# Niccolo-Ajroldi/plainLM

Hardware: AMD Instinct MI355X
Metric: tokens/sec fwd+bwd (160M, seq=1024, bf16) (higher is better)
Workload: dtype bf16

## Files before the change

### plainlm_amd/csrc/gemm_big.hip

```cpp
#include <stdlib.h>

#include <type_traits>
#include <utility>

#include "plm_device.h"

#include <initializer_list>

typedef __attribute__((address_space(3))) void lds_void_t;
typedef const __attribute__((address_space(1))) void gbl_void_t;

__device__ __forceinline__ void big_dma16(const void* gsrc, void* lds_wave_base) {
  __builtin_amdgcn_global_load_lds((gbl_void_t*)gsrc, (lds_void_t*)lds_wave_base, 16, 0, 0);
}
__device__ __forceinline__ int big_swz(int row, int chunk) { return row * 128 + ((chunk ^ ((row >> 1) & 7)) << 4); }

template <int N>
__device__ __forceinline__ void wait_vm() {
#ifdef PLM_DBG_DRAIN
  asm volatile("s_waitcnt vmcnt(0)" ::: "memory");
#else
  asm volatile("s_waitcnt vmcnt(%0)" ::"n"(N) : "memory");
#endif
}
template <int N0, int N1>
__device__ __forceinline__ void wait_vm_sel(int flag) {
#ifdef PLM_DBG_DRAIN
  asm volatile("s_waitcnt vmcnt(0)" ::: "memory");
  return;
#endif
  asm volatile("s_cmp_lg_u32 %0, 0\n\ts_cbranch_scc1 1f\n\ts_waitcnt vmcnt(%1)\n\ts_branch 2f\n1:\n\ts_waitcnt vmcnt(%2)\n2:" ::"s"(flag), "n"(N0), "n"(N1)
               : "memory", "scc");
}
template <int N0, int N1, int N2>
__device__ __forceinline__ void wait_vm_sel3(int flag) {
#ifdef PLM_DBG_DRAIN
  asm volatile("s_waitcnt vmcnt(0)" ::: "memory");
  return;
#endif
  asm volatile("s_cmp_lg_u32 %0, 0\n\ts_cbranch_scc1 1f\n\ts_waitcnt vmcnt(%1)\n\ts_branch 3f\n1:\n\ts_cmp_lg_u32 %0, 1\n\ts_cbranch_scc1 2f\n\ts_waitcnt vmcnt(%2)\n\t"
               "s_branch 3f\n2:\n\ts_waitcnt vmcnt(%3)\n3:" ::"s"(flag), "n"(N0), "n"(N1), "n"(N2)
               : "memory", "scc");
}
__device__ __forceinline__ void phase_barrier() { asm volatile("s_waitcnt lgkmcnt(0)\n\ts_barrier" ::: "memory"); }

#define BIG_GROUP_M 4

static int g_num_cus = 0;
static int g_cu_reserve = 0;

static int persistent_slots() {
  const int n = g_num_cus - g_cu_reserve;
  return n < 8 ? 8 : n;
}

extern "C" int plm_set_cu_reserve(int n) {
  if (n < 0 || n > 128) {
    plm_set_error("plm_set_cu_reserve: n=%d out of range 0..128", n);
    return PLM_E_INVALID;
  }
  g_cu_reserve = n;
  return PLM_OK;
}

static bool ensure_num_cus() {
  if (g_num_cus == 0) {
    int dev = 0;
    hipDeviceProp_t prop;
    if (hipGetDevice(&dev) != hipSuccess || hipGetDeviceProperties(&prop, dev) != hipSuccess) return false;
    g_num_cus = prop.multiProcessorCount > 0 ? prop.multiProcessorCount : 256;
  }
  return true;
}

static double round_efficiency(int64_t tiles, int slots) {
  const int64_t rounds = (tiles + slots - 1) / slots;
  return (double)tiles / (double)(rounds * slots);
}

struct HybridArgs {
  int rfull;
  int nchunks;
  int L;
  float* slabs;
};

struct EpiArgs {
  uint16_t* act;
  int64_t ldact;
  const float* rcos;
  const float* rsin;
  int T, rope_cols;
};

template <class F, int... U>
__device__ __forceinline__ void nt_for_units(F& f, std::integer_sequence<int, U...>) {
  (f(std::integral_constant<int, U>{}), ...);
}
template <int NA, int NBF, int BF0>
struct NtOvlPlan {
  static constexpr int NPASS = (NBF + 1) / 2, NUNIT = NA * NPASS;
  static constexpr int pass_blocks(int u) { const int p0 = (u % NPASS) * 2; return NBF - p0 < 2 ? NBF - p0 : 2; }
  static constexpr int stores(int u) { return 2 * pass_blocks(u); }
  static constexpr int ready(int u) {
    const int mf = u / NPASS, p0 = (u % NPASS) * 2, nb = pass_blocks(u);
    const int h[2] = {(2 * mf) / NA, (2 * mf + 1) / NA};
    const bool b[2] = {p0 < BF0, p0 + nb - 1 >= BF0};
    int r = 0;
    for (int i = 0; i < 2; ++i)
      for (int j = 0; j < 2; ++j)
        if (b[j]) {
          const int ph = h[i] == 0 ? (j == 0 ? 1 : 2) : (j == 1 ? 3 : 4);
          r = ph > r ? ph : r;
        }
    return r;
  }
  static constexpr int slot(int u) {
    bool taken[6] = {false, false, false, false, false, false};
    int slot_u = 5;
    for (int r = 1; r <= 4; ++r)
      for (int v = 0; v < NUNIT; ++v)
        if (ready(v) == r) {
          int sl = 5;
          for (int c = r + 1; c <= 4; ++c)
            if (!taken[c]) {
              sl = c;
              break;
            }
          if (sl < 5) taken[sl] = true;
          if (v == u) slot_u = sl;
        }
    return slot_u;
  }
  static constexpr int stores_in_slot(int sl) {
    int n = 0;
    for (int u = 0; u < NUNIT; ++u)
      if (slot(u) == sl) n += stores(u);
    return n;
  }
  static constexpr int unit_in_slot(int sl) {
    for (int u = 0; u < NUNIT; ++u)
      if (slot(u) == sl) return u;
    return -1;
  }
};
static_assert(NtOvlPlan<2, 3, 2>::slot(0) == 2 && NtOvlPlan<2, 3, 2>::slot(1) == 3 && NtOvlPlan<2, 3, 2>::slot(3) == 4 && NtOvlPlan<2, 3, 2>::slot(2) == 5,
              "256x192: (A0,B0) (A0,B1) (A1,B1) leave in phases 2 3 4, (A1,B0) behind the loop");
static_assert(NtOvlPlan<4, 2, 1>::slot(0) == 3 && NtOvlPlan<4, 2, 1>::slot(1) == 4 && NtOvlPlan<4, 2, 1>::slot(2) == 5 && NtOvlPlan<4, 2, 1>::slot(3) == 5,
              "256x256: the two pieces of A half 0 leave in phases 3 and 4");
static_assert(NtOvlPlan<1, 3, 2>::slot(1) == 4 && NtOvlPlan<1, 3, 2>::slot(0) == 5, "128x192: the B1 pass leaves in phase 4");

template <int BM, int BN, int WM, int WN, bool HYB = false, bool GLU = false, bool GLUB = false, bool ROPE = false>
__global__ __launch_bounds__(512, 2) void gemm_nt_big_kernel(const uint16_t* __restrict__ A, int64_t lda,
                                                             const uint16_t* __restrict__ B, int64_t ldb,
                                                             uint16_t* __restrict__ C, int64_t ldc, int M, int N, int K,
                                                             const float* __restrict__ alpha_dev, int tiles_m, int tiles_n,
                                                             HybridArgs hyb, EpiArgs ea) {
  uint16_t* const act = ea.act;
  const int64_t ldact = ea.ldact;
  static_assert(!(GLU || GLUB) || (BM == 256 && BN == 256 && WN == 4 && !HYB), "GLU epilogues: 256x256 tiles, whole-K items");
  static_assert(!(GLU && GLUB), "one epilogue at a time");
  constexpr int TM = BM / WM, TN = BN / WN;
  static_assert(WM * WN == 8 && (TN == 64 || TN == 96) && (TM == 128 || TM == 64 || TM == 32), "unsupported geometry");
  constexpr int AH = TM / 2;
  constexpr int NA = AH / 16;
  constexpr int BF0 = TN / 32 - 1, NBF = BF0 + 1;
  constexpr int A_ROWS = BM / 2, B0_ROWS = WN * 32 * BF0, B1_ROWS = WN * 32;
  constexpr int A_HT = A_ROWS * 128, B0_HT = B0_ROWS * 128, B1_HT = B1_ROWS * 128;
  constexpr int STAGE = 2 * A_HT + B0_HT + B1_HT;
  constexpr int A_DMA = A_ROWS / 64, B0_DMA = B0_ROWS / 64, B1_DMA = B1_ROWS / 64;
  static_assert(B0_DMA >= B1_DMA && B1_DMA >= 1, "half-tiles are whole DMA rounds of the workgroup");
  constexpr int OFF_A0 = 0, OFF_B0 = A_HT, OFF_B1 = A_HT + B0_HT, OFF_A1 = A_HT + B0_HT + B1_HT;
  constexpr int D_P4 = 2 * A_DMA + B0_DMA + 2 * B1_DMA;
  constexpr int D_P1 = 3 * A_DMA + B0_DMA + B1_DMA;
  constexpr int D_P2 = 3 * A_DMA + B0_DMA + B1_DMA;
  constexpr int NS = NA * 2 * NBF * (GLUB ? 2 : 1) + (GLU ? NA * 2 : 0);
  static_assert(D_P1 + NS < 64, "vmcnt is a 6-bit counter");
#ifndef PLM_NT_OVL
#define PLM_NT_OVL 1
#endif
  constexpr bool OVL = PLM_NT_OVL && !HYB && !GLU && !GLUB && !ROPE;
  using OP = NtOvlPlan<NA, NBF, BF0>;
  constexpr int NPASS = OP::NPASS, NUNIT = OP::NUNIT;
  constexpr int OVS_2 = OVL ? OP::stores_in_slot(2) : 0, OVS_3 = OVL ? OP::stores_in_slot(3) : 0, OVS_4 = OVL ? OP::stores_in_slot(4) : 0;
  static_assert(OVS_2 + OVS_3 + OVS_4 + (OVL ? OP::stores_in_slot(5) : NS) == NS, "every unit has a slot");
  static_assert(D_P4 + NS < 64, "vmcnt is a 6-bit counter");
  __shared__ __attribute__((aligned(1024))) char smem[2 * STAGE + 8 * 4096];

  const int t = threadIdx.x, lane = t & 63;
  const int wave = __builtin_amdgcn_readfirstlane(t >> 6);
  const int wm = wave / WN, wn = wave % WN;
  const bool grp1 = (wave >> 2) != 0;
  if (wave >= 4) __builtin_amdgcn_s_setprio(1);
  const int l15 = lane & 15, q = lane >> 4;
  const int rfull = HYB ? hyb.rfull : tiles_m;
  const int n_full = rfull * tiles_n;
  const int nkt = K / 64;
  const int g_total = HYB ? (tiles_m - rfull) * tiles_n * nkt : 0;
  const int ntiles = n_full + (HYB ? hyb.nchunks : 0);
  char* epi = smem + 2 * STAGE + wave * 4096;

  struct Cur {
    int item, g, gend;
  };
  auto cur_init = [&](Cur& c, int item) {
    c.item = item;
    c.g = c.gend = 0;
    if (HYB && item >= n_full && item < ntiles) {
      c.g = (item - n_full) * hyb.L;
      c.gend = min(g_total, c.g + hyb.L);
    }
  };
  auto take = [&](Cur& c, int& m0, int& n0, int& kbeg, int& kend, int& sidx) {
    if (!HYB || c.item < n_full) {
      const int group_size = BIG_GROUP_M * tiles_n;
      const int group = c.item / group_size;
      const int first_m = group * BIG_GROUP_M;
      const int gm = min(rfull - first_m, BIG_GROUP_M);
      const int in_group = c.item - group * group_size;
      m0 = (first_m + in_group % gm) * BM;
      n0 = (in_group / gm) * BN;
      kbeg = 0;
      kend = K;
      sidx = -1;
      cur_init(c, c.item + gridDim.x);
    } else {
      const int t = c.g / nkt;
      const int k0 = c.g - t * nkt;
      const int k1 = min(nkt, k0 + (c.gend - c.g));
      m0 = (rfull + t / tiles_n) * BM;
      n0 = (t % tiles_n) * BN;
      kbeg = k0 * 64;
      kend = k1 * 64;
      sidx = (c.item - n_full) - (t * nkt) / hyb.L;
      c.g += k1 - k0;
      if (c.g >= c.gend) cur_init(c, c.item + gridDim.x);
    }
  };

  unsigned oa[2][A_DMA], ob[2][B0_DMA];
  const uint16_t* s_ab = A;
  const uint16_t* s_bb = B;
  const uint16_t* s_ak = A;
  const uint16_t* s_bk = B;
  auto set_ptrs = [&](int m0, int n0) {
    s_ab = A + (int64_t)m0 * lda;
    s_bb = B + (int64_t)(GLU ? n0 / 2 : n0) * ldb;
#pragma unroll
    for (int h = 0; h < 2; ++h) {
#pragma unroll
      for (int i = 0; i < A_DMA; ++i) {
        const int r = (i * 8 + wave) * 8 + (lane >> 3);
        const int chunk = (lane & 7) ^ ((r >> 1) & 7);
        const int m = min((r / AH) * TM + h * AH + (r % AH), M - 1 - m0);
        oa[h][i] = (unsigned)(((int64_t)m * lda + chunk * 8) * 2);
      }
#pragma unroll
      for (int i = 0; i < (h ? B1_DMA : B0_DMA); ++i) {
        const int r = (i * 8 + wave) * 8 + (lane >> 3);
        const int chunk = (lane & 7) ^ ((r >> 1) & 7);
        const int rw = h ? 32 : 32 * BF0;
        const int n = GLU ? h * (N / 2) + r : min((r / rw) * TN + h * 32 * BF0 + (r % rw), N - 1 - n0);
        ob[h][i] = (unsigned)(((int64_t)n * ldb + chunk * 8) * 2);
      }
    }
  };
  auto issue_a = [&](int h, char* stage, int k0) {
    char* dst = stage + (h ? OFF_A1 : OFF_A0);
#pragma unroll
    for (int i = 0; i < A_DMA; ++i) {
      (void)k0;
      big_dma16(reinterpret_cast<const char*>(s_ak) + oa[h][i], dst + (i * 8 + wave) * 1024);
    }
  };
  auto issue_b = [&](int h, char* stage, int k0) {
    char* dst = stage + (h ? OFF_B1 : OFF_B0);
#pragma unroll
    for (int i = 0; i < B0_DMA; ++i) {
      if (i >= (h ? B1_DMA : B0_DMA)) continue;
      (void)k0;
      big_dma16(reinterpret_cast<const char*>(s_bk) + ob[h][i], dst + (i * 8 + wave) * 1024);
    }
  };
  auto frag16 = [&](const char* ht, int row, int ks) -> bf16x8_t {
    return *reinterpret_cast<const bf16x8_t*>(ht + big_swz(row, ks * 4 + q));
  };

  const int first = xcd_remap(blockIdx.x, gridDim.x);
  if (first >= ntiles) return;
  Cur sc;
  cur_init(sc, first);
  int s_k = 0, s_kend = 0;
  int s_item = first;
  auto open_piece = [&]() {
    s_item = sc.item;
    if (s_item < ntiles) {
      int m0, n0, sp_;
      take(sc, m0, n0, s_k, s_kend, sp_);
      set_ptrs(m0, n0);
      s_ak = s_ab + s_k;
      s_bk = s_bb + s_k;
    } else {
      s_k -= 64;
      s_ak -= 64;
      s_bk -= 64;
    }
  };
  int s_st = 0;
  auto advance_staged = [&]() {
    s_k += 64;
    s_ak += 64;
    s_bk += 64;
    s_st ^= 1;
    if (s_k >= s_kend) open_piece();
  };
  open_piece();

  float alpha = alpha_dev ? *alpha_dev : 1.f;
  asm volatile("; alpha pinned" : "+v"(alpha));

  {
    issue_a(0, smem, s_k);
    issue_b(0, smem, s_k);
    issue_b(1, smem, s_k);
    issue_a(1, smem, s_k);
    advance_staged();
  }
  {
    issue_a(0, smem + STAGE, s_k);
    issue_b(0, smem + STAGE, s_k);
    issue_b(1, smem + STAGE, s_k);
    wait_vm<D_P4>();
  }
  phase_barrier();

  int st = 0;
  bool credit = false;
  int credit_i = 0;
  Cur cc;
  cur_init(cc, first);
  while (cc.item < ntiles) {
    int m0 = 0, n0 = 0, kbeg = 0, kend = K, split = -1;
    if (HYB) take(cc, m0, n0, kbeg, kend, split);
    const int nk = HYB ? (kend - kbeg) / 64 : nkt;
    f32x4_t acc4[2 * NA][2 * NBF];
#pragma unroll
    for (int i = 0; i < 2 * NA; ++i)
#pragma unroll
      for (int j = 0; j < 2 * NBF; ++j)
#pragma unroll
        for (int r = 0; r < 4; ++r) acc4[i][j][r] = 0.f;

    auto unit_write = [&](auto utag) {
      constexpr int u = decltype(utag)::value, mf = u / NPASS, p0 = (u % NPASS) * 2, nb = OP::pass_blocks(u);
#pragma unroll
      for (int bq = 0; bq < nb; ++bq) {
        const int bh = p0 + bq;
#pragma unroll
        for (int sr = 0; sr < 2; ++sr)
#pragma unroll
          for (int sc = 0; sc < 2; ++sc) {
            bf16x4_t o;
#pragma unroll
            for (int e = 0; e < 4; ++e) o[e] = f2bf(acc4[2 * mf + sr][bh * 2 + sc][e]);
            const int row = sr * 16 + l15, c = bq * 4 + sc * 2 + (q >> 1);
            *reinterpret_cast<bf16x4_t*>(epi + row * 128 + ((c ^ (row & 7)) << 4) + (q & 1) * 8) = o;
          }
      }
    };
    auto unit_store = [&](auto utag, auto interior, int m0, int n0) {
      constexpr int u = decltype(utag)::value, mf = u / NPASS, p0 = (u % NPASS) * 2, nb = OP::pass_blocks(u);
      const int mrow0 = m0 + wm * TM + mf * 32;
      bf16x8_t v[2 * nb];
#pragma unroll
      for (int it = 0; it < 2 * nb; ++it) {
        const int c = it * 64 + lane;
        const int row = nb == 2 ? c >> 3 : c >> 2, ch = nb == 2 ? c & 7 : c & 3;
        v[it] = *reinterpret_cast<const bf16x8_t*>(epi + row * 128 + ((ch ^ (row & 7)) << 4));
      }
#pragma unroll
      for (int it = 0; it < 2 * nb; ++it) {
        const int c = it * 64 + lane;
        const int row = nb == 2 ? c >> 3 : c >> 2, ch = nb == 2 ? c & 7 : c & 3;
        const int gm = mrow0 + row;
        const int gn = n0 + wn * TN + p0 * 32 + ch * 8;
        if (decltype(interior)::value || (gm < M && gn < N)) st_c_bf16x8(C + (int64_t)gm * ldc + gn, v[it]);
      }
    };

    auto ktile = [&](auto lasttag, int m0, int n0) {
      constexpr bool LASTOVL = decltype(lasttag)::value;
      const char* cur = smem + st * STAGE;
      bf16x8_t a6[NA][2], b06[2 * BF0][2], b16[2][2];
      auto end_phase = [&](auto wtag, auto w2tag) {
        constexpr int W = decltype(wtag)::value, W2 = decltype(w2tag)::value;
        if (LASTOVL) wait_vm<W>();
        else if (OVL) wait_vm_sel3<W, W + NS, W + W2>(credit_i);
        else wait_vm_sel<W, W + NS>(credit_i);
        phase_barrier();
      };
      using std::integral_constant;
      auto slot_write = [&](auto sltag) {
        constexpr int u = OP::unit_in_slot(decltype(sltag)::value);
        if constexpr (LASTOVL && u >= 0) unit_write(integral_constant<int, (u >= 0 ? u : 0)>{});
      };
      auto slot_store = [&](auto sltag) {
        constexpr int u = OP::unit_in_slot(decltype(sltag)::value);
        if constexpr (LASTOVL && u >= 0) {
          asm volatile("s_waitcnt lgkmcnt(0)" ::: "memory");
          unit_store(integral_constant<int, (u >= 0 ? u : 0)>{}, std::true_type{}, m0, n0);
        }
      };
      constexpr int S2 = LASTOVL ? OVS_2 : 0, S4 = LASTOVL ? OVS_2 + OVS_3 + OVS_4 : 0;

      issue_a(1, smem + s_st * STAGE, s_k);
      advance_staged();
#pragma unroll
      for (int ks = 0; ks < 2; ++ks) {
#pragma unroll
        for (int j = 0; j < 2 * BF0; ++j) b06[j][ks] = frag16(cur + OFF_B0, wn * BF0 * 32 + j * 16 + l15, ks);
#pragma unroll
        for (int f = 0; f < NA; ++f) a6[f][ks] = frag16(cur + OFF_A0, wm * AH + f * 16 + l15, ks);
      }
      if (grp1) end_phase(integral_constant<int, D_P1>{}, integral_constant<int, NS>{});
#pragma unroll
      for (int ks = 0; ks < 2; ++ks)
#pragma unroll
        for (int f = 0; f < NA; ++f)
#pragma unroll
          for (int j = 0; j < 2 * BF0; ++j) acc4[f][j] = mfma16(b06[j][ks], a6[f][ks], acc4[f][j]);
      if (!grp1) end_phase(integral_constant<int, D_P1>{}, integral_constant<int, NS>{});

      issue_a(0, smem + s_st * STAGE, s_k);
#pragma unroll
      for (int ks = 0; ks < 2; ++ks)
#pragma unroll
        for (int c = 0; c < 2; ++c) b16[c][ks] = frag16(cur + OFF_B1, wn * 32 + c * 16 + l15, ks);
      slot_write(integral_constant<int, 2>{});
      if (grp1) end_phase(integral_constant<int, D_P2>{}, integral_constant<int, NS>{});
#pragma unroll
      for (int ks = 0; ks < 2; ++ks)
#pragma unroll
        for (int f = 0; f < NA; ++f)
#pragma unroll
          for (int c = 0; c < 2; ++c) acc4[f][2 * BF0 + c] = mfma16(b16[c][ks], a6[f][ks], acc4[f][2 * BF0 + c]);
      slot_store(integral_constant<int, 2>{});
      if (!grp1) end_phase(integral_constant<int, D_P2 + S2>{}, integral_constant<int, NS>{});

      issue_b(0, smem + s_st * STAGE, s_k);
#pragma unroll
      for (int ks = 0; ks < 2; ++ks)
#pragma unroll
        for (int f = 0; f < NA; ++f) a6[f][ks] = frag16(cur + OFF_A1, wm * AH + f * 16 + l15, ks);
      slot_write(integral_constant<int, 3>{});
      if (grp1) end_phase(integral_constant<int, D_P4 - B1_DMA + S2>{}, integral_constant<int, NS - OVS_2>{});
#pragma unroll
      for (int ks = 0; ks < 2; ++ks)
#pragma unroll
        for (int f = 0; f < NA; ++f)
#pragma unroll
          for (int c = 0; c < 2; ++c) acc4[NA + f][2 * BF0 + c] = mfma16(b16[c][ks], a6[f][ks], acc4[NA + f][2 * BF0 + c]);
      slot_store(integral_constant<int, 3>{});

      issue_b(1, smem + s_st * STAGE, s_k);
      slot_write(integral_constant<int, 4>{});
#pragma unroll
      for (int ks = 0; ks < 2; ++ks)
#pragma unroll
        for (int f = 0; f < NA; ++f)
#pragma unroll
          for (int j = 0; j < 2 * BF0; ++j) acc4[NA + f][j] = mfma16(b06[j][ks], a6[f][ks], acc4[NA + f][j]);
      slot_store(integral_constant<int, 4>{});
      if (!grp1) end_phase(integral_constant<int, D_P4 + S4>{}, integral_constant<int, NS - OVS_2>{});
      credit = false;
      credit_i = 0;
      st ^= 1;
    };

    bool ovl = false;
    if (OVL) {
      Cur peek = cc;
      int pm0, pn0, pk0, pk1, psp;
      take(peek, pm0, pn0, pk0, pk1, psp);
      ovl = __builtin_amdgcn_readfirstlane(nk >= 2 && alpha_dev == nullptr && pm0 + BM <= M && pn0 + BN <= N);
    }
    {
      const int nloop = ovl ? nk - 1 : nk;
      for (int kt = 0; kt < nloop; ++kt) ktile(std::false_type{}, 0, 0);
    }
    if (OVL && ovl) {
      Cur peek = cc;
      int pm0, pn0, pk0, pk1, psp;
      take(peek, pm0, pn0, pk0, pk1, psp);
      ktile(std::true_type{}, pm0, pn0);
    }

    if (!HYB) take(cc, m0, n0, kbeg, kend, split);
    if (HYB && split >= 0) {
      const int mrem = M - rfull * BM;
      float* slab = hyb.slabs + ((int64_t)split * mrem - (int64_t)rfull * BM) * N;
#pragma unroll
      for (int f = 0; f < 2 * NA; ++f) {
        const int gm = m0 + wm * TM + f * 16 + l15;
        if (gm >= M) continue;
#pragma unroll
        for (int j = 0; j < 2 * NBF; ++j) {
          const int gn = n0 + wn * TN + j * 16 + 4 * q;
          if (gn >= N) continue;
          *reinterpret_cast<f32x4_t*>(slab + (int64_t)gm * N + gn) = acc4[f][j];
        }
      }
      continue;
    }
    if (HYB || alpha_dev != nullptr) {
#pragma unroll
      for (int i = 0; i < 2 * NA; ++i)
#pragma unroll
        for (int j = 0; j < 2 * NBF; ++j) acc4[i][j] *= alpha;
    }
    if constexpr (OVL) {
      auto drain = [&](auto utag) {
        constexpr int u = decltype(utag)::value;
        if (ovl && OP::slot(u) != 5) return;
        unit_write(utag);
        asm volatile("s_waitcnt lgkmcnt(0)" ::: "memory");
        unit_store(utag, std::false_type{}, m0, n0);
        asm volatile("s_waitcnt lgkmcnt(0)" ::: "memory");
      };
      nt_for_units(drain, std::make_integer_sequence<int, NUNIT>{});
      credit = m0 + BM <= M && n0 + BN <= N;
      credit_i = __builtin_amdgcn_readfirstlane(credit ? (ovl ? 2 : 1) : 0);
      continue;
    }
#pragma unroll
    for (int mf = 0; mf < NA; ++mf) {
      const int mrow0 = m0 + wm * TM + mf * 32;
      if (GLUB) {
        const uint16_t* u = act;
#pragma unroll
        for (int sr = 0; sr < 2; ++sr) {
          const int gm_l = min(mrow0 + sr * 16 + l15, M - 1);
          const int fi = 2 * mf + sr;
#pragma unroll
          for (int bq = 0; bq < 2; ++bq)
#pragma unroll
            for (int sc = 0; sc < 2; ++sc) {
              const int gn = n0 + wn * TN + bq * 32 + sc * 16 + 4 * q;
              const bf16x4_t xv = ld_bf16x4(u + (int64_t)gm_l * ldact + gn);
              const bf16x4_t zv = ld_bf16x4(u + (int64_t)gm_l * ldact + N + gn);
              bf16x4_t dxo, dzo;
#pragma unroll
              for (int e = 0; e < 4; ++e) {
                const float gf = bf2f(f2bf(acc4[fi][bq * 2 + sc][e]));
                const float xf = bf2f(xv[e]), zf = bf2f(zv[e]);
                const float sig = plm_sigmoid(xf);
                const bf16_t sv = f2bf(xf * sig);
                const bf16_t ds = f2bf(gf * zf);
                dzo[e] = f2bf(gf * bf2f(sv));
                dxo[e] = f2bf(bf2f(ds) * (sig * (1.f + xf * (1.f - sig))));
              }
              const int c = bq * 4 + sc * 2 + (q >> 1);
              *reinterpret_cast<bf16x4_t*>(epi + l15 * 128 + ((c ^ (l15 & 7)) << 4) + (q & 1) * 8) = dxo;
              *reinterpret_cast<bf16x4_t*>(epi + (16 + l15) * 128 + ((c ^ (l15 & 7)) << 4) + (q & 1) * 8) = dzo;
            }
          asm volatile("s_waitcnt lgkmcnt(0)" ::: "memory");
#pragma unroll
          for (int it = 0; it < 4; ++it) {
            const int c = it * 64 + lane;
            const int row = c >> 3, ch = c & 7;
            const bf16x8_t v = *reinterpret_cast<const bf16x8_t*>(epi + row * 128 + ((ch ^ (row & 7)) << 4));
            const int gm = mrow0 + sr * 16 + (row & 15);
            if (gm < M) st_c2_bf16x8(C + (int64_t)gm * ldc + (row >> 4) * N + n0 + wn * TN + ch * 8, v);
          }
          asm volatile("s_waitcnt lgkmcnt(0)" ::: "memory");
        }
        continue;
      }
#pragma unroll
      for (int p0 = 0; p0 < NBF; p0 += 2) {
        const int nb = NBF - p0 < 2 ? NBF - p0 : 2;
#pragma unroll
        for (int bq = 0; bq < 2; ++bq) {
          if (bq >= nb) continue;
          const int bh = p0 + bq;
#pragma unroll
          for (int sr = 0; sr < 2; ++sr)
#pragma unroll
            for (int sc = 0; sc < 2; ++sc) {
              bf16x4_t o;
#pragma unroll
              for (int e = 0; e < 4; ++e) o[e] = f2bf(acc4[2 * mf + sr][bh * 2 + sc][e]);
              const int row = sr * 16 + l15, c = bq * 4 + sc * 2 + (q >> 1);
              *reinterpret_cast<bf16x4_t*>(epi + row * 128 + ((c ^ (row & 7)) << 4) + (q & 1) * 8) = o;
            }
        }
        asm volatile("s_waitcnt lgkmcnt(0)" ::: "memory");
#pragma unroll
        for (int it = 0; it < 4; ++it) {
          if (it >= 2 * nb) continue;
          const int c = it * 64 + lane;
          const int row = nb == 2 ? c >> 3 : c >> 2, ch = nb == 2 ? c & 7 : c & 3;
          const bf16x8_t v = *reinterpret_cast<const bf16x8_t*>(epi + row * 128 + ((ch ^ (row & 7)) << 4));
          const int gm = mrow0 + row;
          const int gn = GLU ? (ch >> 2) * (N / 2) + n0 / 2 + wn * 32 + (ch & 3) * 8 : n0 + wn * TN + p0 * 32 + ch * 8;
          if (ROPE) {
            if (gm < M && gn < ea.rope_cols) {
              const int tab = (gm % ea.T) * 32 + ((gn & 63) >> 1);
              st_c2_bf16x8(C + (int64_t)gm * ldc + gn, rope8(v, *reinterpret_cast<const f32x4_t*>(ea.rcos + tab),
                                                          *reinterpret_cast<const f32x4_t*>(ea.rsin + tab), 1.f));
              continue;
            }
          }
          if (gm < M && gn < N) st_c_bf16x8(C + (int64_t)gm * ldc + gn, v);
        }
        asm volatile("s_waitcnt lgkmcnt(0)" ::: "memory");
      }
      if (GLU) {
#pragma unroll
        for (int sr = 0; sr < 2; ++sr)
#pragma unroll
          for (int sc = 0; sc < 2; ++sc) {
            const int fi = 2 * mf + sr;
            bf16x4_t o;
#pragma unroll
            for (int e = 0; e < 4; ++e) o[e] = plm_swiglu_bf16(f2bf(acc4[fi][sc][e]), f2bf(acc4[fi][2 + sc][e]));
            const int row = sr * 16 + l15, c = sc * 2 + (q >> 1);
            *reinterpret_cast<bf16x4_t*>(epi + row * 128 + ((c ^ (row & 7)) << 4) + (q & 1) * 8) = o;
          }
        asm volatile("s_waitcnt lgkmcnt(0)" ::: "memory");
#pragma unroll
        for (int it = 0; it < 2; ++it) {
          const int c = it * 64 + lane;
          const int row = c >> 2, ch = c & 3;
          const bf16x8_t v = *reinterpret_cast<const bf16x8_t*>(epi + row * 128 + ((ch ^ (row & 7)) << 4));
          const int gm = mrow0 + row;
          if (gm < M) st_c2_bf16x8(act + (int64_t)gm * ldact + n0 / 2 + wn * 32 + ch * 8, v);
        }
        asm volatile("s_waitcnt lgkmcnt(0)" ::: "memory");
      }
    }
    credit = m0 + BM <= M && n0 + BN <= N;
    credit_i = __builtin_amdgcn_readfirstlane(credit ? 1 : 0);
  }
  wait_vm<0>();
}

#define PLM_TN_GROUP_MAX 48
struct TnGroup {
  const uint16_t* A[PLM_TN_GROUP_MAX];
  const uint16_t* B[PLM_TN_GROUP_MAX];
  int lda[PLM_TN_GROUP_MAX], ldb[PLM_TN_GROUP_MAX];
  int M[PLM_TN_GROUP_MAX], N[PLM_TN_GROUP_MAX], tiles_n[PLM_TN_GROUP_MAX];
  int tile_base[PLM_TN_GROUP_MAX + 1];
  int count;
  int n_full;
  int splits;
  int L;
};
struct TnGroupOut {
  float* C[PLM_TN_GROUP_MAX];
  const float* alpha[PLM_TN_GROUP_MAX];
  int ldc[PLM_TN_GROUP_MAX];
  int accumulate[PLM_TN_GROUP_MAX];
};

__device__ __forceinline__ int tn_rot(int k) { return 2 * (k & 3) + ((k >> 3) & 1); }

template <bool GROUPED = false>
__global__ __launch_bounds__(512, 2) void gemm_tn_big_kernel(const uint16_t* __restrict__ A, int64_t lda,
                                                             const uint16_t* __restrict__ B, int64_t ldb, float* __restrict__ C,
                                                             int64_t ldc, float* __restrict__ slabs, int M, int N, int K, int kchunk,
                                                             int splits, int rfull, int accumulate,
                                                             const float* __restrict__ alpha_dev, int tiles_m, int tiles_n, TnGroup grp,
                                                             TnGroupOut gout) {
  constexpr int BM = 256, BN = 256, WN = 4;
  constexpr int TM = 128, TN = 64, AH = 64, AF = 2, NA = 2 * AF;
  constexpr int HT = 64 * 256;
  constexpr int STAGE = 4 * HT;
  constexpr int OFF_A0 = 0, OFF_B0 = HT, OFF_B1 = 2 * HT, OFF_A1 = 3 * HT;
  constexpr int W_ALL = 10;
  __shared__ __attribute__((aligned(1024))) char smem[2 * STAGE];

  const int t = threadIdx.x, lane = t & 63;
  const int wave = __builtin_amdgcn_readfirstlane(t >> 6);
  const int wm = wave / WN, wn = wave % WN;
  const bool grp1 = (wave >> 2) != 0;
#ifndef PLM_NO_PRIO_HALF_TN
  if (wave >= 4) __builtin_amdgcn_s_setprio(1);
#endif
  const int t16 = lane & 15;
  const int q = lane >> 4;
  const int n_full = rfull * tiles_n;
  const int n_rem = tiles_m * tiles_n - n_full;
  const int nkt = K / 64;
  const int g_ntl = GROUPED ? grp.tile_base[grp.count] : 0, g_nrem = GROUPED ? g_ntl - grp.n_full : 0;
  const int nitems = GROUPED ? grp.n_full + g_nrem * grp.splits : n_full + n_rem * splits;
  int c_prob = 0, c_tile = 0;

  auto coords = [&](int item, int& i0, int& j0, int& kbeg, int& kend, int& split) {
    int tile;
    if (GROUPED) {
      int t, lo, hi2;
      if (item < grp.n_full) {
        split = -1;
        t = item;
        lo = 0;
        hi2 = nkt;
      } else {
        const int j = item - grp.n_full;
        split = j / g_nrem;
        t = grp.n_full + (j - split * g_nrem);
        lo = min(nkt, split * grp.L);
        hi2 = min(nkt, (split + 1) * grp.L);
      }
      kbeg = kend = 0;
      i0 = j0 = 0;
      if (hi2 <= lo) return;
      t = __builtin_amdgcn_readfirstlane(t);
      int pidx = 0;
#pragma unroll
      for (int q = 1; q < PLM_TN_GROUP_MAX; ++q)
        if (q < grp.count && t >= grp.tile_base[q]) pidx = q;
      pidx = __builtin_amdgcn_readfirstlane(pidx);
      const int local = t - grp.tile_base[pidx];
      i0 = (local / grp.tiles_n[pidx]) * BM;
      j0 = (local % grp.tiles_n[pidx]) * BN;
      kbeg = lo * 64;
      kend = hi2 * 64;
      c_prob = pidx;
      c_tile = t;
      return;
    }
    if (item < n_full) {
      split = -1;
      tile = item;
      kbeg = 0;
      kend = K;
    } else {
      const int j = item - n_full;
      split = j / n_rem;
      tile = n_full + (j - split * n_rem);
      kbeg = min(K, split * kchunk);
      kend = min(K, kbeg + kchunk);
    }
    i0 = (tile / tiles_n) * BM;
    j0 = (tile % tiles_n) * BN;
  };

  unsigned pa[2][2], pb[2][2];
  const uint16_t* s_ap = A;
  const uint16_t* s_bp = B;
  int64_t s_lda = lda, s_ldb = ldb;
  auto set_ptrs = [&](int item) {
    int i0, j0, kbeg, kend, split;
    coords(item, i0, j0, kbeg, kend, split);
    const uint16_t* Ap = GROUPED ? grp.A[c_prob] : A;
    const uint16_t* Bp = GROUPED ? grp.B[c_prob] : B;
    const int Mp = GROUPED ? grp.M[c_prob] : M, Np = GROUPED ? grp.N[c_prob] : N;
    if (GROUPED) {
      s_lda = (int64_t)grp.lda[c_prob];
      s_ldb = (int64_t)grp.ldb[c_prob];
    }
    s_ap = Ap;
    s_bp = Bp;
#pragma unroll
    for (int i = 0; i < 2; ++i) {
      const int row = (i * 8 + wave) * 4 + (lane >> 4);
      const int pp = (lane & 15) >> 1, half16 = lane & 1;
      const int cb = (pp - tn_rot(row)) & 7;
      const int c = cb * 16 + half16 * 8;
#pragma unroll
      for (int h = 0; h < 2; ++h) {
        const int ci = i0 + (c / AH) * TM + h * AH + (c % AH);
        const int cj = j0 + (c / 32) * TN + h * 32 + (c % 32);
        pa[h][i] = (unsigned)(((int64_t)row * s_lda + min(ci, Mp - 8)) * 2);
        pb[h][i] = (unsigned)(((int64_t)row * s_ldb + min(cj, Np - 8)) * 2);
      }
    }
  };
  const unsigned smem_u = __builtin_amdgcn_readfirstlane(lds_addr_u32(smem));
  auto issue = [&](const uint16_t* base, const unsigned (&off)[2], int64_t ld, unsigned dst, int k0) {
    const uint16_t* kb = base + (int64_t)k0 * ld;
#pragma unroll
    for (int i = 0; i < 2; ++i) dma16_saddr_u32(kb, off[i], dst + (i * 8 + wave) * 1024);
  };
  auto tr_frag16 = [&](const char* ht, int c0, int ks) -> bf16x8_t {
    const int row = ks * 32 + q * 8 + (t16 >> 2);
    const char* p = ht + row * 256 + (((c0 >> 4) + tn_rot(row)) & 7) * 32 + (t16 & 3) * 8;
    return join_tr(lds_read_tr16(p), lds_read_tr16(p + 4 * 256));
  };

  const int first = xcd_remap(blockIdx.x, gridDim.x);
  if (first >= nitems) return;
  float alpha = alpha_dev ? *alpha_dev : 1.f;
  asm volatile("; alpha pinned" : "+v"(alpha));

  int s_item = first, s_k = 0, s_kend = 0;
  auto open_item = [&]() {
    while (s_item < nitems) {
      int i0, j0, kbeg, kend, split;
      coords(s_item, i0, j0, kbeg, kend, split);
      if (kend > kbeg) {
        s_k = kbeg;
        s_kend = kend;
        set_ptrs(s_item);
        return;
      }
      s_item += gridDim.x;
    }
  };
  int s_st = 0;
  auto advance_staged = [&]() {
    s_k += 64;
    s_st ^= 1;
    if (s_k >= s_kend) {
      s_item += gridDim.x;
      open_item();
    }
  };
  open_item();
  if (s_item < nitems) {
    issue(s_ap, pa[0], s_lda, smem_u + OFF_A0, s_k);
    issue(s_bp, pb[0], s_ldb, smem_u + OFF_B0, s_k);
    issue(s_bp, pb[1], s_ldb, smem_u + OFF_B1, s_k);
    issue(s_ap, pa[1], s_lda, smem_u + OFF_A1, s_k);
    advance_staged();
  }
  if (s_item < nitems) {
    issue(s_ap, pa[0], s_lda, smem_u + STAGE + OFF_A0, s_k);
    issue(s_bp, pb[0], s_ldb, smem_u + STAGE + OFF_B0, s_k);
    issue(s_bp, pb[1], s_ldb, smem_u + STAGE + OFF_B1, s_k);
    wait_vm<W_ALL>();
  } else {
    wait_vm<0>();
// ... 549 lines not shown
```

Before: 1.066 million.

## Defer last epilogue unit store into next tile's first k-iteration

In the overlapped persistent GEMM, the epilogue unit in slot 5 was written to LDS and stored after the k-loop. It is now packed into bf16 registers and carried over to the next tile, where its LDS write and global store are issued during the first k-tile's MFMA phase. The vmcnt wait thresholds for that first k-tile are adjusted to account for the deferred stores. This hides tail epilogue latency behind compute, at the cost of extra live registers and more complex counter bookkeeping.

```diff
diff --git a/plainlm_amd/csrc/gemm_big.hip b/plainlm_amd/csrc/gemm_big.hip
--- a/plainlm_amd/csrc/gemm_big.hip
+++ b/plainlm_amd/csrc/gemm_big.hip
@@ -184,6 +184,13 @@
   constexpr int NPASS = OP::NPASS, NUNIT = OP::NUNIT;
   constexpr int OVS_2 = OVL ? OP::stores_in_slot(2) : 0, OVS_3 = OVL ? OP::stores_in_slot(3) : 0, OVS_4 = OVL ? OP::stores_in_slot(4) : 0;
   static_assert(OVS_2 + OVS_3 + OVS_4 + (OVL ? OP::stores_in_slot(5) : NS) == NS, "every unit has a slot");
+#ifndef PLM_NT_DEFER
+#define PLM_NT_DEFER 1
+#endif
+  constexpr int DU = OVL ? OP::unit_in_slot(5) : -1;
+  constexpr bool DEFER = PLM_NT_DEFER && OVL && DU >= 0 && OP::stores_in_slot(5) == OP::stores(DU < 0 ? 0 : DU);
+  constexpr int DS = DEFER ? OP::stores(DU) : 0;
+  constexpr int DNB = DEFER ? OP::pass_blocks(DU) : 1;
   static_assert(D_P4 + NS < 64, "vmcnt is a 6-bit counter");
   __shared__ __attribute__((aligned(1024))) char smem[2 * STAGE + 8 * 4096];
 
@@ -337,6 +344,8 @@
   int st = 0;
   bool credit = false;
   int credit_i = 0;
+  bf16x4_t dpk[DNB * 4];
+  int dpend = 0, dm0 = 0, dn0 = 0;
   Cur cc;
   cur_init(cc, first);
   while (cc.item < ntiles) {
@@ -351,21 +360,48 @@
 #pragma unroll
         for (int r = 0; r < 4; ++r) acc4[i][j][r] = 0.f;
 
+    auto unit_pack = [&](auto utag, bf16x4_t* o) {
+      constexpr int u = decltype(utag)::value, mf = u / NPASS, p0 = (u % NPASS) * 2, nb = OP::pass_blocks(u);
+#pragma unroll
+      for (int bq = 0; bq < nb; ++bq)
+#pragma unroll
+        for (int sr = 0; sr < 2; ++sr)
+#pragma unroll
+          for (int sc = 0; sc < 2; ++sc)
+#pragma unroll
+            for (int e = 0; e < 4; ++e) o[(bq * 2 + sr) * 2 + sc][e] = f2bf(acc4[2 * mf + sr][(p0 + bq) * 2 + sc][e]);
+    };
+    auto unit_put = [&](auto utag, const bf16x4_t* o) {
+      constexpr int nb = OP::pass_blocks(decltype(utag)::value);
+#pragma unroll
+      for (int bq = 0; bq < nb; ++bq)
+#pragma unroll
+        for (int sr = 0; sr < 2; ++sr)
+#pragma unroll
+          for (int sc = 0; sc < 2; ++sc) {
+            const int row = sr * 16 + l15, c = bq * 4 + sc * 2 + (q >> 1);
+            *reinterpret_cast<bf16x4_t*>(epi + row * 128 + ((c ^ (row & 7)) << 4) + (q & 1) * 8) = o[(bq * 2 + sr) * 2 + sc];
+          }
+    };
     auto unit_write = [&](auto utag) {
       constexpr int u = decltype(utag)::value, mf = u / NPASS, p0 = (u % NPASS) * 2, nb = OP::pass_blocks(u);
-#pragma unroll
-      for (int bq = 0; bq < nb; ++bq) {
-        const int bh = p0 + bq;
-#pragma unroll
-        for (int sr = 0; sr < 2; ++sr)
-#pragma unroll
-          for (int sc = 0; sc < 2; ++sc) {
-            bf16x4_t o;
-#pragma unroll
-            for (int e = 0; e < 4; ++e) o[e] = f2bf(acc4[2 * mf + sr][bh * 2 + sc][e]);
-            const int row = sr * 16 + l15, c = bq * 4 + sc * 2 + (q >> 1);
-            *reinterpret_cast<bf16x4_t*>(epi + row * 128 + ((c ^ (row & 7)) << 4) + (q & 1) * 8) = o;
-          }
+      if constexpr (DEFER) {
+        bf16x4_t o[4 * nb];
+        unit_pack(utag, o);
+        unit_put(utag, o);
+      } else {
+#pragma unroll
+        for (int bq = 0; bq < nb; ++bq)
+#pragma unroll
+          for (int sr = 0; sr < 2; ++sr)
+#pragma unroll
+            for (int sc = 0; sc < 2; ++sc) {
+              bf16x4_t o;
+#pragma unroll
+              for (int e = 0; e < 4; ++e) o[e] = f2bf(acc4[2 * mf + sr][(p0 + bq) * 2 + sc][e]);
+              const int row = sr * 16 + l15, c = bq * 4 + sc * 2 + (q >> 1);
+              *reinterpret_cast<bf16x4_t*>(epi + row * 128 + ((c ^ (row & 7)) << 4) + (q & 1) * 8) = o;
+            }
       }
     };
     auto unit_store = [&](auto utag, auto interior, int m0, int n0) {
@@ -388,13 +424,15 @@
       }
     };
 
-    auto ktile = [&](auto lasttag, int m0, int n0) {
+    auto ktile = [&](auto lasttag, auto deftag, int m0, int n0) {
       constexpr bool LASTOVL = decltype(lasttag)::value;
+      constexpr bool FIRSTDEF = decltype(deftag)::value;
       const char* cur = smem + st * STAGE;
       bf16x8_t a6[NA][2], b06[2 * BF0][2], b16[2][2];
       auto end_phase = [&](auto wtag, auto w2tag) {
         constexpr int W = decltype(wtag)::value, W2 = decltype(w2tag)::value;
         if (LASTOVL) wait_vm<W>();
+        else if (FIRSTDEF) wait_vm<W + W2>();
         else if (OVL) wait_vm_sel3<W, W + NS, W + W2>(credit_i);
         else wait_vm_sel<W, W + NS>(credit_i);
         phase_barrier();
@@ -422,13 +460,18 @@
 #pragma unroll
         for (int f = 0; f < NA; ++f) a6[f][ks] = frag16(cur + OFF_A0, wm * AH + f * 16 + l15, ks);
       }
-      if (grp1) end_phase(integral_constant<int, D_P1>{}, integral_constant<int, NS>{});
+      if constexpr (FIRSTDEF) unit_put(integral_constant<int, (DU >= 0 ? DU : 0)>{}, dpk);
+      if (grp1) end_phase(integral_constant<int, D_P1>{}, integral_constant<int, NS - (FIRSTDEF ? DS : 0)>{});
 #pragma unroll
       for (int ks = 0; ks < 2; ++ks)
 #pragma unroll
         for (int f = 0; f < NA; ++f)
 #pragma unroll
           for (int j = 0; j < 2 * BF0; ++j) acc4[f][j] = mfma16(b06[j][ks], a6[f][ks], acc4[f][j]);
+      if constexpr (FIRSTDEF) {
+        asm volatile("s_waitcnt lgkmcnt(0)" ::: "memory");
+        unit_store(integral_constant<int, (DU >= 0 ? DU : 0)>{}, std::true_type{}, dm0, dn0);
+      }
       if (!grp1) end_phase(integral_constant<int, D_P1>{}, integral_constant<int, NS>{});
 
       issue_a(0, smem + s_st * STAGE, s_k);
@@ -486,13 +529,19 @@
     }
     {
       const int nloop = ovl ? nk - 1 : nk;
-      for (int kt = 0; kt < nloop; ++kt) ktile(std::false_type{}, 0, 0);
+      int kt = 0;
+      if (DEFER && dpend) {
+        ktile(std::false_type{}, std::true_type{}, 0, 0);
+        dpend = 0;
+        kt = 1;
+      }
+      for (; kt < nloop; ++kt) ktile(std::false_type{}, std::false_type{}, 0, 0);
     }
     if (OVL && ovl) {
       Cur peek = cc;
       int pm0, pn0, pk0, pk1, psp;
       take(peek, pm0, pn0, pk0, pk1, psp);
-      ktile(std::true_type{}, pm0, pn0);
+      ktile(std::true_type{}, std::false_type{}, pm0, pn0);
     }
 
     if (!HYB) take(cc, m0, n0, kbeg, kend, split);
@@ -519,9 +568,16 @@
         for (int j = 0; j < 2 * NBF; ++j) acc4[i][j] *= alpha;
     }
     if constexpr (OVL) {
+      const bool defer = DEFER && ovl && cc.item < ntiles;
       auto drain = [&](auto utag) {
         constexpr int u = decltype(utag)::value;
         if (ovl && OP::slot(u) != 5) return;
+        if constexpr (DEFER && u == DU) {
+          if (defer) {
+            unit_pack(utag, dpk);
+            return;
+          }
+        }
         unit_write(utag);
         asm volatile("s_waitcnt lgkmcnt(0)" ::: "memory");
         unit_store(utag, std::false_type{}, m0, n0);
@@ -530,6 +586,11 @@
       nt_for_units(drain, std::make_integer_sequence<int, NUNIT>{});
       credit = m0 + BM <= M && n0 + BN <= N;
       credit_i = __builtin_amdgcn_readfirstlane(credit ? (ovl ? 2 : 1) : 0);
+      if (DEFER) {
+        dpend = __builtin_amdgcn_readfirstlane(defer ? 1 : 0);
+        dm0 = m0;
+        dn0 = n0;
+      }
       continue;
     }
 #pragma unroll
```

Measured after the change: 1.065 million (median of 6 runs). No clear change (-0.1%).
